# Chain123/RecGURU

Measured on AMD Instinct MI355X. Metric: user-sequences/sec (AE+GAN step), higher is better.
Workload: dtype bf16; 1 GPU; cross-domain RecGURU AE+GAN phase-2 iteration (5 critic + 1 generator update), two 100000-item domains; per_gpu_batch=4096, seq_len=200, d_model=128, n_head=4, n_blocks=3, d_ff=512, n_negs=30, user_lengths=U{5..220}, parallelism=dp1

## Files before the change

### include/recguru_hip.h

```cpp
#ifndef RECGURU_HIP_H
#define RECGURU_HIP_H
#include <stddef.h>
#include <stdint.h>
#ifdef __cplusplus
extern "C" {
#endif

#define RG_F32 0
#define RG_BF16 1
#define RG_X3 2

#define RG_ERR_INVALID (-1)
#define RG_ERR_UNSUPPORTED (-2)
#define RG_ERR_HIP (-3)

const char* rg_last_error(void);
int rg_version(void);

int rg_det_enabled(void);
int rg_det_set_arenas(void* fbase0, void* sbase0, unsigned long long bytes0, int bits0,
                      void* fbase1, void* sbase1, unsigned long long bytes1, int bits1);
int rg_det_fault(int clear);

#define RG_PRO_NONE 0
// ... 189 lines not shown
#define RG_CAST_SPLIT 4
int rg_cast(const float* src, void* dst, int R, int C, int transpose, int dtype, void* stream);
typedef struct {
  const float* src; void* dst;
  int R, C, ld, row_off, col_off, transpose;
} rg_cast_seg;
int rg_cast_multi(const rg_cast_seg* segs , const int* tiles , int ntiles,
                  int dtype, void* stream);

#define RG_LOSS_SAMPLED_CE 0
#define RG_LOSS_BPR 1
#define RG_LOSS_BPR_SAS 2
typedef struct {
  const void* h;
  const void* table;
  const int64_t* pos;
  const int64_t* neg;
  const float* mask;
  float* aux_tok;
  float* sums;
  const float* gout;
  void* dh; float* dE;
  long long ntok; int d; int k; int mode; long long skip_row;
} rg_item_loss_args;
int rg_item_loss_fwd(const rg_item_loss_args* args , int dtype, void* stream);
int rg_item_loss_bwd(const rg_item_loss_args* args , int dtype, void* stream);
size_t rg_item_loss_bwd_binned_workspace(long long ntok, int k, int d, long long table_rows);
int rg_item_loss_bwd_binned(const rg_item_loss_args* args , long long table_rows, void* workspace,
                            size_t workspace_bytes, int dtype, void* stream);
int rg_item_loss_train_supported(int k, int d);
int rg_item_loss_train(const rg_item_loss_args* args , float* coef, int dtype, void* stream);
int rg_item_loss_scatter_binned(const rg_item_loss_args* args , const float* coef, long long table_rows,
                                void* workspace, size_t workspace_bytes, int dtype, void* stream);
typedef struct {
  const void* h;
  const void* w;
  const int64_t* labels;
  const float* mask;
  const int* live16;
  float* lse;
  void* dh;
  float* partials;
  float* sums;
  const float* gout;
  float* dw;
  long long n; long long C; int d;
} rg_full_ce_args;
int rg_full_ce_supported(int d, int dtype);
int rg_full_ce_fwd(const rg_full_ce_args* args , int train, int dtype, void* stream);
int rg_full_ce_dw(const rg_full_ce_args* args , int dtype, void* stream);
typedef struct {
  const void* h;
  const void* table;
  const int64_t* labels;
  const int64_t* cand;
  const float* mask;
  const int* live16;
  const float* cand_bias;
  const float* pos_bias;
  void* wc;
  float* lse;
  void* dh;
  float* coef_pos;
  float* partials;
  float* sums;
  const float* gout;
// ... 174 lines not shown
```

### recguru_amd/csrc/loss.hip

```cpp
#include <stdlib.h>
#include "rg_common.hip.h"
#include "rg_det.hip.h"
#include "../../include/recguru_hip.h"

#define LW 4

#define RG_SAS_EPS 1e-24f
__device__ __forceinline__ float sigmoidf_(float x) { return 1.f / (1.f + __expf(-x)); }
__device__ __forceinline__ void bpr_value(int mode, float p, float nbar, float& loss, float& aux) {
  if (mode == RG_LOSS_BPR_SAS) {
    aux = nbar;
    loss = -(__logf(sigmoidf_(p) + RG_SAS_EPS) + __logf(1.f - sigmoidf_(nbar) + RG_SAS_EPS));
  } else {
    aux = p - nbar;
    loss = -__logf(sigmoidf_(aux));
  }
}
__device__ __forceinline__ float bpr_coef(int mode, int idx, float aux, float p, int k) {
  if (mode == RG_LOSS_BPR_SAS) {
    if (idx == 0) { const float sp = sigmoidf_(p); return -sp * (1.f - sp) / (sp + RG_SAS_EPS); }
    const float sn = sigmoidf_(aux);
    return sn * (1.f - sn) / (1.f - sn + RG_SAS_EPS) / (float)k;
  }
  const float sg = 1.f / (1.f + __expf(aux));
// ... 469 lines not shown
template <typename T>
static int launch(const rg_item_loss_args& a, bool bwd, hipStream_t s) {
  long long g = (a.ntok + LW - 1) / LW;
  if (g > 256 * 32) g = 256 * 32;
  dim3 grid((int)g), block(64 * LW);
#define RG_R(LPR)                                                                             \
  do {                                                                                        \
    if (bwd) hipLaunchKernelGGL((item_loss_bwd_rows_kernel<T, LPR, false>), grid, block, 0, s, a, (float*)nullptr);   \
    else hipLaunchKernelGGL((item_loss_fwd_rows_kernel<T, LPR>), grid, block, 0, s, a);       \
    RG_CHECK_LAUNCH();                                                                        \
    return 0;                                                                                 \
  } while (0)
  if (a.d == 64) RG_R(8);
  if (a.d == 128) RG_R(16);
  if (a.d == 256) RG_R(32);
#undef RG_R
#define RG_L(NPL)                                                                   \
  if (bwd) hipLaunchKernelGGL((item_loss_bwd_kernel<T, NPL>), grid, block, 0, s, a); \
  else hipLaunchKernelGGL((item_loss_fwd_kernel<T, NPL>), grid, block, 0, s, a)
  if (a.d <= 64) { RG_L(1); }
  else if (a.d <= 128) { RG_L(2); }
  else if (a.d <= 256) { RG_L(4); }
  else return rg_set_error_msg(RG_ERR_UNSUPPORTED, "item_loss: d > 256");
#undef RG_L
  RG_CHECK_LAUNCH();
  return 0;
}

#define RG_RPB 64
#define RG_RPB_LOG 6
#define RG_CHUNK 2048
#define RG_CHUNK_EMB 512
#define RG_MAXBINS 8192
#define RG_PPW 8192
#define RG_PPW_WIDE 65536

struct BinWs {
  float* c; int* hist; int* start; int* cursor; int* chunk_start;
  int* chunk_bin;
  int chunk;
  uint2* ent;
  int nbins;
  int ppw;
  int bin_log;
  const float* cscale;
  const float* lse;
  const float* count;
};

#define RG_PB 4
__device__ __forceinline__ void pair_items4(const rg_item_loss_args& a, long long p, long long p1, int n, long long (&it)[RG_PB]) {
  float mk[RG_PB];
#pragma unroll
  for (int u = 0; u < RG_PB; ++u) {
    const long long pc = min(p + 256 * u, p1 - 1);
    const long long t = (long long)((unsigned int)pc / (unsigned int)n);
    const int idx = (int)(pc - t * n);
    mk[u] = a.mask[t];
    const int64_t* __restrict__ src = idx == 0 ? a.pos + t : a.neg + t * a.k + (idx - 1);
    it[u] = *src;
  }
#pragma unroll
  for (int u = 0; u < RG_PB; ++u)
    if (p + 256 * u >= p1 || mk[u] == 0.f || it[u] == a.skip_row) it[u] = -1;
}

__global__ __launch_bounds__(256) void bin_count_kernel(rg_item_loss_args a, BinWs w) {
  extern __shared__ int lh[];
  const int n = a.k + 1;
  const long long npairs = a.ntok * n;
  for (int i = threadIdx.x; i < w.nbins; i += 256) lh[i] = 0;
  __syncthreads();
  const long long p0 = (long long)blockIdx.x * w.ppw, p1 = min(p0 + w.ppw, npairs);
  for (long long p = p0 + threadIdx.x; p < p1; p += 256 * RG_PB) {
    long long it[RG_PB];
    pair_items4(a, p, p1, n, it);
#pragma unroll
    for (int u = 0; u < RG_PB; ++u)
      if (it[u] >= 0) atomicAdd(&lh[it[u] >> w.bin_log], 1);
  }
  __syncthreads();
  for (int i = threadIdx.x; i < w.nbins; i += 256)
    if (lh[i]) atomicAdd(&w.hist[i], lh[i]);
}

__global__ __launch_bounds__(1024) void bin_scan_kernel(BinWs w) {
  __shared__ int wt[16], wtc[16];
  const int tid = threadIdx.x, lane = tid & 63, wv = tid >> 6;
  const int per = (w.nbins + 1023) / 1024;
  const int b0 = tid * per, b1 = min(b0 + per, w.nbins);
  int s = 0, sc = 0;
  for (int b = b0; b < b1; ++b) { s += w.hist[b]; sc += (w.hist[b] + w.chunk - 1) / w.chunk; }
  int is = s, isc = sc;
#pragma unroll
  for (int o = 1; o < 64; o <<= 1) {
    const int u = __shfl_up(is, o), uc = __shfl_up(isc, o);
    if (lane >= o) { is += u; isc += uc; }
  }
  if (lane == 63) { wt[wv] = is; wtc[wv] = isc; }
  __syncthreads();
  int base = 0, basec = 0;
  for (int i = 0; i < wv; ++i) { base += wt[i]; basec += wtc[i]; }
  if (tid == 1023) { w.start[w.nbins] = base + is; w.chunk_start[w.nbins] = basec + isc; }
  s = base + is - s; sc = basec + isc - sc;
  for (int b = b0; b < b1; ++b) {
    w.start[b] = s; w.cursor[b] = s; w.chunk_start[b] = sc;
    const int nc = (w.hist[b] + w.chunk - 1) / w.chunk;
    for (int j = 0; j < nc; ++j) w.chunk_bin[sc + j] = b;
    s += w.hist[b]; sc += nc;
  }
}

__global__ __launch_bounds__(256) void bin_fill_kernel(rg_item_loss_args a, BinWs w) {
  extern __shared__ int lh[];
  int* base = lh + w.nbins;
  const int n = a.k + 1;
  const long long npairs = a.ntok * n;
  const float gsc = w.cscale ? w.cscale[0] : 1.f;
  for (int i = threadIdx.x; i < w.nbins; i += 256) lh[i] = 0;
  __syncthreads();
  const long long p0 = (long long)blockIdx.x * w.ppw, p1 = min(p0 + w.ppw, npairs);
  for (long long p = p0 + threadIdx.x; p < p1; p += 256 * RG_PB) {
    long long it[RG_PB];
    pair_items4(a, p, p1, n, it);
#pragma unroll
    for (int u = 0; u < RG_PB; ++u)
      if (it[u] >= 0) atomicAdd(&lh[it[u] >> w.bin_log], 1);
  }
  __syncthreads();
  for (int i = threadIdx.x; i < w.nbins; i += 256) {
    const int cnt = lh[i];
    base[i] = cnt ? atomicAdd(&w.cursor[i], cnt) : 0;
    lh[i] = 0;
  }
  __syncthreads();
  for (long long p = p0 + threadIdx.x; p < p1; p += 256 * RG_PB) {
    long long it[RG_PB];
    float cv[RG_PB];
    pair_items4(a, p, p1, n, it);
#pragma unroll
    for (int u = 0; u < RG_PB; ++u) cv[u] = w.c[min(p + 256 * u, p1 - 1)];
    if (w.lse) {
      const float ic = 1.f / w.count[0];
#pragma unroll
      for (int u = 0; u < RG_PB; ++u) {
        const long long pc = min(p + 256 * u, p1 - 1);
        const long long t = (long long)((unsigned int)pc / (unsigned int)n);
        cv[u] = (__expf(cv[u] - w.lse[t]) - (pc - t * n == 0 ? 1.f : 0.f)) * a.mask[t] * ic;
      }
    }
#pragma unroll
    for (int u = 0; u < RG_PB; ++u) cv[u] *= gsc;
#pragma unroll
    for (int u = 0; u < RG_PB; ++u) {
      if (it[u] < 0) continue;
      const long long pu = p + 256 * u;
      const int b = (int)(it[u] >> w.bin_log);
      const int e = base[b] + atomicAdd(&lh[b], 1);
      w.ent[e] = make_uint2((((unsigned int)pu / (unsigned int)n) << w.bin_log) | (unsigned int)(it[u] & ((1 << w.bin_log) - 1)), __float_as_uint(cv[u]));
    }
  }
}

template <typename T, int LPR, bool DROP>
__global__ __launch_bounds__(256) void bin_accumulate_kernel(rg_item_loss_args a, BinWs w, long long table_rows, DropCfg drop) {
  constexpr int CH = DROP ? RG_CHUNK_EMB : RG_CHUNK;
  constexpr int G = 64 / LPR, D = LPR * 8, U = 4, EPT = CH / 256;
  extern __shared__ float sm[];
  float* acc = sm;
  int* st = reinterpret_cast<int*>(sm + RG_RPB * D);
  float* sc = reinterpret_cast<float*>(st + CH);
  __shared__ int cnt[RG_RPB], rstart[RG_RPB + 1];
// ... 252 lines not shown
        for (int u = 0; u < U; ++u)
#pragma unroll
          for (int j = 0; j < 8; ++j) s8[j] += c[u] * h[u][j];
      }
#pragma unroll
      for (int o = LPR; o < 64; o <<= 1)
#pragma unroll
        for (int j = 0; j < 8; ++j) s8[j] += __shfl_xor(s8[j], o);
      if (gi == 0) store8(myrow + 8 * li, s8);
      __builtin_amdgcn_fence(__ATOMIC_RELEASE, "wavefront");
      __builtin_amdgcn_wave_barrier();
      const long long row = (long long)bin * RB + r;
      if (row < table_rows) {
        float* __restrict__ dst = a.dE + row * D;
#pragma unroll
        for (int i = 0; i < D / 64; ++i) {
          const float v = myrow[lane + 64 * i];
          if (v != 0.f) { if (alone) dst[lane + 64 * i] += v; else atomicAdd(dst + lane + 64 * i, v); }
        }
      }
      __builtin_amdgcn_wave_barrier();
    }
    __syncthreads();
  }
}

static size_t align256(size_t x) { return (x + 255) & ~(size_t)255; }

static int bin_log_of(long long table_rows) {
  if ((table_rows + RG_RPB - 1) / RG_RPB <= RG_MAXBINS) return RG_RPB_LOG;
  if ((table_rows + RG_WIDE_RPB - 1) / RG_WIDE_RPB <= RG_MAXBINS) return RG_WIDE_LOG;
  return 0;
}
extern "C" size_t rg_item_loss_bwd_binned_workspace(long long ntok, int k, int d, long long table_rows) {
  if (RG_DET) return 0;
  const int bl = bin_log_of(table_rows);
  if (!bl) return 0;
  const long long nbins = (table_rows + (1LL << bl) - 1) >> bl;
  const long long npairs = ntok * (k + 1);
  if (!(d == 64 || d == 128 || d == 256) || npairs >= (1LL << 31) || ntok <= 0 || ntok >= (1LL << (32 - bl))) return 0;
  return align256(npairs * 4) + align256(npairs * 8) + align256((nbins + 1) * 4) * 4 + align256((nbins + npairs / RG_CHUNK_EMB + 1) * 4);
}

template <typename T>
static int launch_binned(const rg_item_loss_args& a, const float* coef, void* ws, size_t ws_bytes, long long table_rows, hipStream_t s,
                         const DropCfg* drop = nullptr) {
  const int n = a.k + 1;
  const long long npairs = a.ntok * n;
  const size_t need = rg_item_loss_bwd_binned_workspace(a.ntok, a.k, a.d, table_rows);
  if (!need) return rg_set_error_msg(RG_ERR_UNSUPPORTED, "item_loss_bwd_binned: needs d in {64,128,256}, <= 8192 bins of 64 (or 256) rows, < 2^31 pairs, < 2^26 (2^24) positions");
  if (!ws || ws_bytes < need) return rg_set_error_msg(RG_ERR_INVALID, "item_loss_bwd_binned: workspace too small");
  BinWs w;
  w.bin_log = bin_log_of(table_rows);
  const bool wide = w.bin_log == RG_WIDE_LOG;
  if (wide && drop) return rg_set_error_msg(RG_ERR_UNSUPPORTED, "embed_scatter_bwd_binned: tables of more than 524288 rows take the atomic form");
  w.nbins = (int)((table_rows + (1LL << w.bin_log) - 1) >> w.bin_log);
  char* p = reinterpret_cast<char*>(ws);
  w.c = coef ? const_cast<float*>(coef) : reinterpret_cast<float*>(p); p += align256(npairs * 4);
  w.cscale = coef ? a.gout : nullptr;
  w.lse = coef ? a.aux_tok : nullptr;
  w.count = a.sums ? a.sums + 1 : nullptr;
  if (w.lse && !w.count) return rg_set_error_msg(RG_ERR_INVALID, "item_loss_scatter_binned: aux_tok (lse of raw logits) needs sums");
  w.chunk = drop ? RG_CHUNK_EMB : (wide ? RG_CHUNK_WIDE : RG_CHUNK);
  w.ent = reinterpret_cast<uint2*>(p); p += align256(npairs * 8);
  const size_t ib = align256((size_t)(w.nbins + 1) * 4);
  w.hist = reinterpret_cast<int*>(p); p += ib;
  w.start = reinterpret_cast<int*>(p); p += ib;
  w.cursor = reinterpret_cast<int*>(p); p += ib;
  w.chunk_start = reinterpret_cast<int*>(p); p += ib;
  w.chunk_bin = reinterpret_cast<int*>(p);
  hipError_t e = hipMemsetAsync(w.hist, 0, ib, s);
  if (e != hipSuccess) return rg_set_error(e, "item_loss_bwd_binned(memset)");
  long long g = (a.ntok + LW - 1) / LW;
  if (g > 256 * 32) g = 256 * 32;
  if (coef) {}
  else if (a.d == 64) hipLaunchKernelGGL((item_loss_bwd_rows_kernel<T, 8, true>), dim3((int)g), dim3(64 * LW), 0, s, a, w.c);
  else if (a.d == 128) hipLaunchKernelGGL((item_loss_bwd_rows_kernel<T, 16, true>), dim3((int)g), dim3(64 * LW), 0, s, a, w.c);
  else hipLaunchKernelGGL((item_loss_bwd_rows_kernel<T, 32, true>), dim3((int)g), dim3(64 * LW), 0, s, a, w.c);
  w.ppw = w.nbins > 4096 ? RG_PPW_WIDE : RG_PPW;
  const int gp = (int)((npairs + w.ppw - 1) / w.ppw);
  hipLaunchKernelGGL(bin_count_kernel, dim3(gp), dim3(256), (size_t)w.nbins * 4, s, a, w);
  hipLaunchKernelGGL(bin_scan_kernel, dim3(1), dim3(1024), 0, s, w);
  hipFuncSetAttribute(reinterpret_cast<const void*>(bin_fill_kernel), hipFuncAttributeMaxDynamicSharedMemorySize, w.nbins * 8);
  hipLaunchKernelGGL(bin_fill_kernel, dim3(gp), dim3(256), (size_t)w.nbins * 8, s, a, w);
  if (wide) {
    const size_t smw = (size_t)RG_CHUNK_WIDE * 8 + (size_t)4 * a.d * 4;
#define RG_ACCW(LPR)                                                                                                 \
  do {                                                                                                               \
    hipFuncSetAttribute(reinterpret_cast<const void*>(bin_accumulate_wide_kernel<T, LPR>), hipFuncAttributeMaxDynamicSharedMemorySize, (int)smw); \
    hipLaunchKernelGGL((bin_accumulate_wide_kernel<T, LPR>), dim3(256 * 2), dim3(256), smw, s, a, w, table_rows);      \
  } while (0)
    if (a.d == 64) RG_ACCW(8);
    else if (a.d == 128) RG_ACCW(16);
    else RG_ACCW(32);
#undef RG_ACCW
    RG_CHECK_LAUNCH();
    return 0;
  }
  const size_t smem = (size_t)RG_RPB * a.d * 4 + (size_t)(drop ? RG_CHUNK_EMB : RG_CHUNK) * 8;
  const int ga = 256 * (int)(smem <= 40 * 1024 ? 4 : (smem <= 52 * 1024 ? 3 : (smem <= 80 * 1024 ? 2 : 1)));
#define RG_ACC1(LPR, DR)                                                                                            \
  do {                                                                                                              \
    hipFuncSetAttribute(reinterpret_cast<const void*>(bin_accumulate_kernel<T, LPR, DR>), hipFuncAttributeMaxDynamicSharedMemorySize, (int)smem); \
    hipLaunchKernelGGL((bin_accumulate_kernel<T, LPR, DR>), dim3(ga), dim3(256), smem, s, a, w, table_rows, dc);      \
  } while (0)
#define RG_ACC(LPR) do { if (drop) RG_ACC1(LPR, true); else RG_ACC1(LPR, false); } while (0)
  const DropCfg dc = drop ? *drop : make_drop(0.f, 0);
  if (a.d == 64) RG_ACC(8);
  else if (a.d == 128) RG_ACC(16);
  else RG_ACC(32);
#undef RG_ACC1
#undef RG_ACC
  RG_CHECK_LAUNCH();
  return 0;
}

extern "C" int rg_item_loss_bwd_binned(const rg_item_loss_args* a, long long table_rows, void* workspace, size_t workspace_bytes,
// ... 29 lines not shown
    else if (a.d == 128) hipLaunchKernelGGL((item_loss_train_online2_kernel<T, 16>), grid, block, 0, s, a, coef);
    else hipLaunchKernelGGL((item_loss_train_online2_kernel<T, 32>), grid, block, 0, s, a, coef);
    RG_CHECK_LAUNCH();
    return 0;
  }
#define RG_TR(LPR)                                                                                           \
  do {                                                                                                       \
    if (nit == 1) hipLaunchKernelGGL((item_loss_train_rows_kernel<T, LPR, 1>), grid, block, 0, s, a, coef);  \
    else if (nit == 2) hipLaunchKernelGGL((item_loss_train_rows_kernel<T, LPR, 2>), grid, block, 0, s, a, coef); \
    else hipLaunchKernelGGL((item_loss_train_rows_kernel<T, LPR, 4>), grid, block, 0, s, a, coef);           \
  } while (0)
  if (a.d == 64) RG_TR(8);
  else if (a.d == 128) RG_TR(16);
  else RG_TR(32);
#undef RG_TR
  RG_CHECK_LAUNCH();
  return 0;
}

extern "C" int rg_item_loss_train(const rg_item_loss_args* a, float* coef, int dtype, void* stream) {
  if (!a || a->ntok <= 0) return 0;
  if (dtype == RG_BF16) return launch_train<__bf16>(*a, coef, (hipStream_t)stream);
  if (dtype == RG_F32) return launch_train<float>(*a, coef, (hipStream_t)stream);
  return rg_set_error_msg(RG_ERR_INVALID, "item_loss_train: bad dtype");
}

extern "C" int rg_item_loss_scatter_binned(const rg_item_loss_args* a, const float* coef, long long table_rows, void* workspace,
                                           size_t workspace_bytes, int dtype, void* stream) {
  if (!a || a->ntok <= 0) return 0;
  if (!coef || !a->gout) return rg_set_error_msg(RG_ERR_INVALID, "item_loss_scatter_binned: coef and gout are required");
  if (dtype == RG_BF16) return launch_binned<__bf16>(*a, coef, workspace, workspace_bytes, table_rows, (hipStream_t)stream);
  if (dtype == RG_F32) return launch_binned<float>(*a, coef, workspace, workspace_bytes, table_rows, (hipStream_t)stream);
  return rg_set_error_msg(RG_ERR_INVALID, "item_loss_scatter_binned: bad dtype");
}

extern "C" size_t rg_embed_scatter_binned_workspace(long long ntok, int d, long long table_rows) {
  if (bin_log_of(table_rows) != RG_RPB_LOG) return 0;
  return rg_item_loss_bwd_binned_workspace(ntok, 0, d, table_rows);
}
extern "C" int rg_embed_scatter_bwd_binned(const void* dx, const int64_t* ids, const float* mask, float* dE, long long ntok, int d,
                                           long long table_rows, long long skip_row, float drop_p, unsigned long long seed,
                                           void* workspace, size_t workspace_bytes, int dtype, void* stream) {
  if (ntok <= 0) return 0;
  if (!dx || !ids || !mask || !dE) return rg_set_error_msg(RG_ERR_INVALID, "embed_scatter_bwd_binned: dx, ids, mask and dE are required");
  rg_item_loss_args a = {};
  a.h = dx; a.pos = ids; a.mask = mask; a.dE = dE; a.ntok = ntok; a.d = d; a.k = 0; a.skip_row = skip_row;
  const DropCfg drop = make_drop(drop_p, seed);
  if (dtype == RG_BF16) return launch_binned<__bf16>(a, mask, workspace, workspace_bytes, table_rows, (hipStream_t)stream, &drop);
  if (dtype == RG_F32) return launch_binned<float>(a, mask, workspace, workspace_bytes, table_rows, (hipStream_t)stream, &drop);
  return rg_set_error_msg(RG_ERR_INVALID, "embed_scatter_bwd_binned: bad dtype");
}

template <typename T, int LPR>
__global__ __launch_bounds__(64 * LW) void rank_scores_kernel(rg_rank_args a) {
  constexpr int G = 64 / LPR;
  const int lane = threadIdx.x & 63, wave = threadIdx.x >> 6;
  const int gi = lane / LPR, li = lane % LPR;
  const T* __restrict__ H = reinterpret_cast<const T*>(a.h);
  const T* __restrict__ E = reinterpret_cast<const T*>(a.table);
  const int d = a.d, n = a.C + 1;
  for (int b = blockIdx.x * LW + wave; b < a.B; b += gridDim.x * LW) {
    float h[8];
    load8(h, H + (size_t)b * d + 8 * li);
    const long long tgt = a.target[b];
    float s0;
    {
// ... 77 lines not shown
```

### recguru_amd/hip.py

```python
import ctypes
import os

import torch

_HERE = os.path.dirname(os.path.abspath(__file__))
DETERMINISTIC = os.environ.get("RG_DETERMINISTIC", "0") not in ("", "0")
LIB_PATH = os.environ.get("RG_HIP_LIB") or os.path.join(_HERE, "librecguru_hip_det.so" if DETERMINISTIC else "librecguru_hip.so")
_lib = None

F32, BF16, X3 = 0, 1, 2
SPLIT_OPERANDS = False
PRO_NONE, PRO_GELU = 0, 1
EPI_NONE, EPI_RELU, EPI_MUL_POSMASK, EPI_GELU_GRAD, EPI_ADD, EPI_RESID_LN, EPI_DROP_GELU = 0, 1, 2, 3, 4, 5, 6

c_p, c_i, c_f, c_l = ctypes.c_void_p, ctypes.c_int, ctypes.c_float, ctypes.c_int64
c_u64 = ctypes.c_uint64


class GemmNtArgs(ctypes.Structure):
    _fields_ = [("A", c_p), ("lda", c_i), ("W", c_p), ("ldw", c_i), ("bias", c_p), ("C", c_p), ("ldc", c_i),
                ("c_is_f32", c_i), ("M", c_i), ("N", c_i), ("K", c_i), ("prologue", c_i), ("epilogue", c_i),
                ("aux", c_p), ("ldaux", c_i), ("gamma", c_p), ("beta", c_p), ("rowmask", c_p),
                ("rstd_out", c_p), ("ln_eps", c_f), ("debug_ablate", c_i), ("epi_scale", c_f),
                ("epi_nonzero_scale", c_f), ("drop_p", c_f), ("drop_seed", c_u64), ("live16", c_p),
# ... 35 lines not shown
class FfnBwdArgs(ctypes.Structure):
    _fields_ = [("dl2", c_p), ("dz", c_p), ("h1", c_p), ("W2t", c_p), ("W1t", c_p), ("dh1", c_p), ("dy", c_p),
                ("M", c_i), ("d", c_i), ("dff", c_i), ("w_packed", c_i), ("nz_scale", c_f), ("live16", c_p),
                ("ln_dout", c_p), ("ln_out", c_p), ("ln_rstd", c_p), ("ln_gamma", c_p), ("ln_beta", c_p), ("ln_rowmask", c_p),
                ("dl2_out", c_p), ("ln_dgamma", c_p), ("ln_dbeta", c_p), ("ln_partials", c_p),
                ("ln_drop_p", c_f), ("ln_drop_seed", c_u64)]


class AttnOutBwdArgs(ctypes.Structure):
    _fields_ = [("dy", c_p), ("y", c_p), ("rstd", c_p), ("gamma", c_p), ("beta", c_p), ("rowmask", c_p), ("Wot", c_p),
                ("dz", c_p), ("dctx", c_p), ("dgamma", c_p), ("dbeta", c_p), ("ln_partials", c_p),
                ("M", c_i), ("d", c_i), ("P", c_i), ("w_packed", c_i), ("live16", c_p)]


class AttnOutBwdCrossArgs(ctypes.Structure):
    _fields_ = [("dy2", c_p), ("y2", c_p), ("rstd_c", c_p), ("cgamma", c_p), ("cbeta", c_p),
                ("y1", c_p), ("rstd1", c_p), ("gamma1", c_p), ("beta1", c_p), ("rowmask", c_p), ("Wot", c_p),
                ("dy1", c_p), ("dz", c_p), ("dctx", c_p),
                ("dcgamma", c_p), ("dcbeta", c_p), ("dz_colsum", c_p), ("dgamma1", c_p), ("dbeta1", c_p), ("partials", c_p),
                ("M", c_i), ("d", c_i), ("P", c_i), ("w_packed", c_i), ("live16", c_p)]


SYMBOLS = ["rg_last_error", "rg_version", "rg_gemm_nt", "rg_gemm_tn", "rg_attn_fwd", "rg_attn_bwd",
           "rg_embed_pe_fwd", "rg_embed_pe_fwd_rows", "rg_embed_scatter_bwd", "rg_ln_bwd", "rg_bcast_add_ln", "rg_seq_sum", "rg_colsum",
           "rg_outer_posmask", "rg_interpolate", "rg_gp_penalty", "rg_sum", "rg_adam", "rg_cast",
           "rg_item_loss_fwd", "rg_item_loss_bwd", "rg_post_attn_fwd",
           "rg_attn_lastq_fwd", "rg_attn_lastq_bwd",
           "rg_cross_drop_scale", "rg_seq_wsum", "rg_gemm_nt_plan", "rg_gemm_tn_plan", "rg_gemm_tn_workspace", "rg_gemm_tn_layer", "rg_gemm_tn_layer_supported", "rg_gemm_tn_layer_workspace", "rg_ln_bwd_workspace", "rg_cast_multi",
           "rg_item_loss_bwd_binned_workspace", "rg_item_loss_bwd_binned", "rg_adam_multi", "rg_rank_scores",
           "rg_assemble_batch", "rg_sample_negatives", "rg_sample_negatives_alias", "rg_dropout", "rg_cross_rows", "rg_live_tiles",
           "rg_adam_multi_dev", "rg_disc_rows", "rg_disc_supported", "rg_attn_fwd_x_supported", "rg_pad_mask", "rg_last_rows",
           "rg_ffn_bwd_data", "rg_ffn_bwd_data_supported", "rg_ffn_bwd_ln_workspace", "rg_first_live",
           "rg_attn_out_bwd", "rg_attn_out_bwd_workspace", "rg_attn_out_bwd_cross", "rg_attn_out_bwd_cross_workspace",
           "rg_item_loss_train_supported", "rg_item_loss_train", "rg_item_loss_scatter_binned", "rg_scale_dev",
           "rg_attn_lastq_x_supported", "rg_attn_lastq_x_fwd", "rg_attn_lastq_x_bwd", "rg_attn_lastq_xf_fwd", "rg_attn_lastq_xf_bwd",
           "rg_embed_scatter_binned_workspace", "rg_embed_scatter_bwd_binned", "rg_embed_pe_fwd_split", "rg_mse",
           "rg_dropout_gelu", "rg_add_drop_ln", "rg_cross_add_ln", "rg_embed_pe_fwd2",
           "rg_det_enabled", "rg_det_set_arenas", "rg_det_fault",
           "rg_full_ce_supported", "rg_full_ce_fwd", "rg_full_ce_dw",
           "rg_shared_ce_supported", "rg_shared_ce_bwd_workspace", "rg_shared_ce_fwd", "rg_shared_ce_bwd",
           "rg_topk_workspace", "rg_topk_scores", "rg_topk_list_workspace", "rg_topk_list",
           "rg_grad_sqnorm_multi", "rg_adam_multi_dev2",
           "rg_pos_grad_workspace", "rg_pos_grad"]
LOSS_SAMPLED_CE, LOSS_BPR, LOSS_BPR_SAS = 0, 1, 2
c_ll = ctypes.c_longlong


class LnBwdArgs(ctypes.Structure):
    _fields_ = [("dy", c_p), ("y", c_p), ("rstd", c_p), ("gamma", c_p), ("beta", c_p), ("rowmask", c_p),
                ("dz", c_p), ("dgamma", c_p), ("dbeta", c_p), ("M", c_ll), ("N", c_i), ("ld", c_i),
                ("dz_drop", c_p), ("drop_p", c_f), ("drop_seed", c_u64), ("live16", c_p), ("dz_colsum", c_p), ("partials", c_p)]


class ItemLossArgs(ctypes.Structure):
    _fields_ = [("h", c_p), ("table", c_p), ("pos", c_p), ("neg", c_p), ("mask", c_p), ("aux_tok", c_p),
                ("sums", c_p), ("gout", c_p), ("dh", c_p), ("dE", c_p), ("ntok", c_ll), ("d", c_i), ("k", c_i),
                ("mode", c_i), ("skip_row", c_ll)]


def _check_screened(path):
    if os.environ.get("RG_ALLOW_UNSCREENED") or os.environ.get("RG_HIP_LIB"):
        return
    info_path = os.path.join(_HERE, "build", "BUILD_INFO_det.json" if os.path.basename(path) == "librecguru_hip_det.so" else "BUILD_INFO.json")
    try:
        import json
        with open(info_path) as f:
            info = json.load(f)
# ... 855 lines not shown

def item_loss_train_supported(k, d):
    return int(lib().rg_item_loss_train_supported(int(k), int(d)))


@_det_accum(sums="S")
def item_loss_train(h, table, pos, neg, mask, k, mode, sums, lse=None):
    ntok, d = h.shape
    assert h.is_contiguous() and table.is_contiguous() and table.dtype == h.dtype
    assert pos.dtype == torch.int64 and neg.dtype == torch.int64 and pos.numel() == ntok and neg.numel() == ntok * k
    coef = torch.empty(ntok * (k + 1), device=h.device, dtype=torch.float32)
    dh = torch.empty_like(h)
    a = ItemLossArgs(_p(h), _p(table), _p(pos), _p(neg), _p(mask), _p(lse), _p(sums), None, _p(dh), None, ntok, d, k,
                     mode, -1)
    _check(lib().rg_item_loss_train(ctypes.byref(a), _vp(coef), dt_of(h), _stream()), "rg_item_loss_train")
    return coef, dh


def item_loss_scatter_binned(h, table_rows, pos, neg, mask, k, coef, gout, dE, skip_row=-1, lse=None, sums=None):
    ntok, d = h.shape
    need = item_loss_bwd_binned_supported(ntok, k, d, table_rows)
    if not need:
        raise RuntimeError("item_loss_scatter_binned: unsupported shape (d=%d, rows=%d, k=%d)" % (d, table_rows, k))
    ws = _BIN_WS.get(h.device)
    if ws is None or ws.numel() < need:
        ws = torch.empty(need, device=h.device, dtype=torch.uint8)
        _BIN_WS[h.device] = ws
    a = ItemLossArgs(_p(h), None, _p(pos), _p(neg), _p(mask), _p(lse), _p(sums), _p(gout), None, _p(dE), ntok, d, k, 0,
                     skip_row)
    _check(lib().rg_item_loss_scatter_binned(ctypes.byref(a), _vp(coef), c_ll(table_rows), _vp(ws), ctypes.c_size_t(need),
                                             dt_of(h), _stream()), "rg_item_loss_scatter_binned")


class FullCeArgs(ctypes.Structure):
    _fields_ = [("h", c_p), ("w", c_p), ("labels", c_p), ("mask", c_p), ("live16", c_p), ("lse", c_p), ("dh", c_p),
                ("partials", c_p), ("sums", c_p), ("gout", c_p), ("dw", c_p), ("n", c_ll), ("C", c_ll), ("d", c_i)]


def _full_ce_code(h):
    return BF16 if h.dtype == torch.bfloat16 else X3


def full_ce_supported(d, h):
    return bool(lib().rg_full_ce_supported(int(d), _full_ce_code(h)))


def full_ce_fwd(h, w, labels, mask, live, sums, train=True):
    n, d = h.shape
    assert h.is_contiguous() and w.is_contiguous() and w.dtype == h.dtype and w.shape[1] == d
    assert labels.dtype == torch.int64 and labels.numel() == n and mask.dtype == torch.float32 and mask.numel() == n
    lse = torch.empty(n, device=h.device, dtype=torch.float32)
    dh = torch.empty_like(h) if train else None
    partials = torch.empty((n + 15) // 16, device=h.device, dtype=torch.float32)
    a = FullCeArgs(_p(h), _p(w), _p(labels), _p(mask), _p(live), _p(lse), _p(dh), _p(partials), _p(sums), None, None,
                   n, w.shape[0], d)
    _check(lib().rg_full_ce_fwd(ctypes.byref(a), int(bool(train)), _full_ce_code(h), _stream()), "rg_full_ce_fwd")
    return lse, dh


def full_ce_dw(h, w, labels, mask, live, lse, sums, gout, dw):
    n, d = h.shape
    assert dw.dtype == torch.float32 and dw.is_contiguous() and tuple(dw.shape) == tuple(w.shape)
    a = FullCeArgs(_p(h), _p(w), _p(labels), _p(mask), _p(live), _p(lse), None, None, _p(sums), _p(gout), _p(dw),
                   n, w.shape[0], d)
    _check(lib().rg_full_ce_dw(ctypes.byref(a), _full_ce_code(h), _stream()), "rg_full_ce_dw")
    return dw
# ... 514 lines not shown
    return ("attn_fwd_kernel<bf16,x-input>", 4.0 * B * H * L * L * 32 + 2.0 * B * L * d * P3,
            B * L * (d + P3 // 3) * _esize(x) + P3 * d * _esize(x))


def _work_ffn_bwd(dl2, dz, h1, *a, **k):
    src = k["ln"][0] if k.get("ln") is not None else dl2
    M, d = src.shape
    dff = h1.shape[1]
    return ("ffn_bwd_data_kernel<%s>" % _tn(src), 4.0 * M * d * dff,
            M * ((4 if k.get("ln") is not None else 3) * d + 2 * dff) * _esize(src))


def _work_lastq_x_fwd(x, q_last, *a, **k):
    B, L, d = x.shape
    return "attn_lastq_x_fwd_kernel", B * (4 * 2.0 * L * d * 2 + 4 * 2.0 * 32 * d * 2), B * L * d * _esize(x) + 2 * B * d * _esize(x)


def _work_lastq_x_bwd(x, q_last, *a, **k):
    B, L, d = x.shape
    return "attn_lastq_x_bwd_kernel", B * (4 * 2.0 * L * d * 5 + 4 * 2.0 * 32 * d * 3), 2 * B * L * d * _esize(x) + 11 * B * d * _esize(x)


def _work_item_loss_train(h, table, pos, neg, mask, k, mode, *a, **kw):
    n, d = h.shape
    nl = float(mask.sum())
    return ("item_loss_train_rows_kernel", 4.0 * nl * (k + 1) * d,
            nl * (k + 2) * d * _esize(table) + n * d * _esize(table) + nl * (k + 1) * 12 + n * 4)


def _work_item_loss_scatter(h, table_rows, pos, neg, mask, k, coef, gout, dE, *a, **kw):
    n, d = h.shape
    nl = float(mask.sum())
    pairs = nl * (k + 1)
    return "item_loss_scatter_binned_kernel", 2.0 * pairs * d, pairs * (d * _esize(h) + 2 * 12 + 2 * 8)


def _work_gemm_tn_layer(probs):
    fl, by, refs = [], [], []
    for i, pr in enumerate(probs):
        if pr is None:
            continue
        Y, X, dW, colsum, live = pr
        T, N1, N2 = Y.shape[0], Y.shape[1], X.shape[1]
        fl.append(2.0 * T * N1 * N2)
        by.append(T * (N1 + N2) * _esize(Y) + N1 * N2 * 4)
        refs.append(live)
    x3 = any(pr is not None and pr[0].dtype == torch.float32 for pr in probs)
    return "gemm_tn_layer_x3_kernel" if x3 else "gemm_tn_layer_kernel", fl, by, refs


def _work_attn_out_bwd(dy, y, rstd, *a, **k):
    M, d = dy.shape
    return "attn_out_bwd_kernel", 2.0 * M * d * d, 4 * M * d * _esize(dy) + M * 4


def _work_attn_out_bwd_cross(dy2, y2, rstd_c, *a, **k):
    M, d = dy2.shape
    return "attn_out_bwd_cross_kernel", 2.0 * M * d * d, 6 * M * d * _esize(dy2) + 3 * M * 4


def _work_ln_bwd(dy, y, rstd, *a, **k):
    M, N = dy.shape
    return "ln_bwd_kernel", 0.0, 3 * M * N * _esize(dy) + M * 4


def _work_full_ce_fwd(h, w, labels, mask, live, sums, train=True):
    n, d = h.shape
# ... 100 lines not shown
```

Baseline: 880,500 user-sequences/sec.

## Replace atomic bin cursors with per-workgroup count matrix and column scan

For the 64-row bin case, the counting sort now writes each workgroup's per-bin histogram into a matrix. A column-wise exclusive scan over that matrix gives each workgroup fixed offsets, so the fill pass no longer takes global atomics on shared cursors and does not have to recount. Sort kernels use 1024 threads and the pairs-per-workgroup is sized so the matrix stays within a 32 MB cap. A standalone rg_bin_sort entry is also exposed, at the cost of extra workspace and an extra scan launch.

```diff
diff --git a/include/recguru_hip.h b/include/recguru_hip.h
--- a/include/recguru_hip.h
+++ b/include/recguru_hip.h
@@ -245,6 +245,9 @@
 int rg_item_loss_train(const rg_item_loss_args* args , float* coef, int dtype, void* stream);
 int rg_item_loss_scatter_binned(const rg_item_loss_args* args , const float* coef, long long table_rows,
                                 void* workspace, size_t workspace_bytes, int dtype, void* stream);
+int rg_bin_sort(const rg_item_loss_args* args , const float* coef, long long table_rows, int ppw, void* workspace,
+                size_t workspace_bytes, size_t* need, long long* ent_off, long long* start_off, int* nbins, int* bin_log,
+                void* stream);
 typedef struct {
   const void* h;
   const void* w;
diff --git a/recguru_amd/csrc/loss.hip b/recguru_amd/csrc/loss.hip
--- a/recguru_amd/csrc/loss.hip
+++ b/recguru_amd/csrc/loss.hip
@@ -525,11 +525,15 @@
 #define RG_CHUNK 2048
 #define RG_CHUNK_EMB 512
 #define RG_MAXBINS 8192
+#define RG_SORT_T 1024
 #define RG_PPW 8192
+#define RG_MAT_BYTES (32u << 20)
 #define RG_PPW_WIDE 65536
 
 struct BinWs {
-  float* c; int* hist; int* start; int* cursor; int* chunk_start;
+  float* c; int* hist; int* start; int* chunk_start;
+  int* mat;
+  int* cursor;
   int* chunk_bin;
   int chunk;
   uint2* ent;
@@ -542,11 +546,12 @@
 };
 
 #define RG_PB 4
-__device__ __forceinline__ void pair_items4(const rg_item_loss_args& a, long long p, long long p1, int n, long long (&it)[RG_PB]) {
-  float mk[RG_PB];
-#pragma unroll
-  for (int u = 0; u < RG_PB; ++u) {
-    const long long pc = min(p + 256 * u, p1 - 1);
+template <int NT, int PB>
+__device__ __forceinline__ void pair_items(const rg_item_loss_args& a, long long p, long long p1, int n, long long (&it)[PB]) {
+  float mk[PB];
+#pragma unroll
+  for (int u = 0; u < PB; ++u) {
+    const long long pc = min(p + NT * u, p1 - 1);
     const long long t = (long long)((unsigned int)pc / (unsigned int)n);
     const int idx = (int)(pc - t * n);
     mk[u] = a.mask[t];
@@ -554,11 +559,61 @@
     it[u] = *src;
   }
 #pragma unroll
-  for (int u = 0; u < RG_PB; ++u)
-    if (p + 256 * u >= p1 || mk[u] == 0.f || it[u] == a.skip_row) it[u] = -1;
-}
-
-__global__ __launch_bounds__(256) void bin_count_kernel(rg_item_loss_args a, BinWs w) {
+  for (int u = 0; u < PB; ++u)
+    if (p + NT * u >= p1 || mk[u] == 0.f || it[u] == a.skip_row) it[u] = -1;
+}
+
+__global__ __launch_bounds__(RG_SORT_T) void bin_count_kernel(rg_item_loss_args a, BinWs w) {
+  extern __shared__ int lh[];
+  const int n = a.k + 1;
+  const long long npairs = a.ntok * n;
+  for (int i = threadIdx.x; i < w.nbins; i += RG_SORT_T) lh[i] = 0;
+  __syncthreads();
+  const long long p0 = (long long)blockIdx.x * w.ppw, p1 = min(p0 + w.ppw, npairs);
+  for (long long p = p0 + threadIdx.x; p < p1; p += RG_SORT_T * RG_PB) {
+    long long it[RG_PB];
+    pair_items<RG_SORT_T, RG_PB>(a, p, p1, n, it);
+#pragma unroll
+    for (int u = 0; u < RG_PB; ++u)
+      if (it[u] >= 0) atomicAdd(&lh[it[u] >> RG_RPB_LOG], 1);
+  }
+  __syncthreads();
+  int* __restrict__ row = w.mat + (size_t)blockIdx.x * w.nbins;
+  for (int i = threadIdx.x; i < w.nbins; i += RG_SORT_T) row[i] = lh[i];
+}
+
+#define RG_CS_BINS 8
+#define RG_CS_SEG 128
+__global__ __launch_bounds__(RG_CS_BINS * RG_CS_SEG) void bin_colscan_kernel(BinWs w, int nwg) {
+  __shared__ int tot[RG_CS_SEG][RG_CS_BINS];
+  const int bl = threadIdx.x % RG_CS_BINS, sg = threadIdx.x / RG_CS_BINS;
+  const int b = blockIdx.x * RG_CS_BINS + bl;
+  const bool live = b < w.nbins;
+  const int per = (nwg + RG_CS_SEG - 1) / RG_CS_SEG;
+  const int r0 = min(sg * per, nwg), r1 = min(r0 + per, nwg);
+  int* __restrict__ col = w.mat + b;
+  int s = 0;
+  if (live)
+    for (int r = r0; r < r1; ++r) s += col[(size_t)r * w.nbins];
+  tot[sg][bl] = s;
+  __syncthreads();
+  int run = 0;
+  for (int i = 0; i < sg; ++i) run += tot[i][bl];
+  if (live) {
+    int r = r0;
+    for (; r + 8 <= r1; r += 8) {
+      int v[8];
+#pragma unroll
+      for (int u = 0; u < 8; ++u) v[u] = col[(size_t)(r + u) * w.nbins];
+#pragma unroll
+      for (int u = 0; u < 8; ++u) { col[(size_t)(r + u) * w.nbins] = run; run += v[u]; }
+    }
+    for (; r < r1; ++r) { const int v = col[(size_t)r * w.nbins]; col[(size_t)r * w.nbins] = run; run += v; }
+    if (sg == RG_CS_SEG - 1) w.hist[b] = run;
+  }
+}
+
+__global__ __launch_bounds__(256) void bin_count_wide_kernel(rg_item_loss_args a, BinWs w) {
   extern __shared__ int lh[];
   const int n = a.k + 1;
   const long long npairs = a.ntok * n;
@@ -567,7 +622,7 @@
   const long long p0 = (long long)blockIdx.x * w.ppw, p1 = min(p0 + w.ppw, npairs);
   for (long long p = p0 + threadIdx.x; p < p1; p += 256 * RG_PB) {
     long long it[RG_PB];
-    pair_items4(a, p, p1, n, it);
+    pair_items<256, RG_PB>(a, p, p1, n, it);
 #pragma unroll
     for (int u = 0; u < RG_PB; ++u)
       if (it[u] >= 0) atomicAdd(&lh[it[u] >> w.bin_log], 1);
@@ -597,14 +652,51 @@
   if (tid == 1023) { w.start[w.nbins] = base + is; w.chunk_start[w.nbins] = basec + isc; }
   s = base + is - s; sc = basec + isc - sc;
   for (int b = b0; b < b1; ++b) {
-    w.start[b] = s; w.cursor[b] = s; w.chunk_start[b] = sc;
+    w.start[b] = s; w.chunk_start[b] = sc;
+    if (w.cursor) w.cursor[b] = s;
     const int nc = (w.hist[b] + w.chunk - 1) / w.chunk;
     for (int j = 0; j < nc; ++j) w.chunk_bin[sc + j] = b;
     s += w.hist[b]; sc += nc;
   }
 }
 
-__global__ __launch_bounds__(256) void bin_fill_kernel(rg_item_loss_args a, BinWs w) {
+__global__ __launch_bounds__(RG_SORT_T) void bin_fill_kernel(rg_item_loss_args a, BinWs w) {
+  extern __shared__ int lh[];
+  const int n = a.k + 1;
+  const long long npairs = a.ntok * n;
+  const float gsc = w.cscale ? w.cscale[0] : 1.f;
+  const int* __restrict__ row = w.mat + (size_t)blockIdx.x * w.nbins;
+  for (int i = threadIdx.x; i < w.nbins; i += RG_SORT_T) lh[i] = w.start[i] + row[i];
+  __syncthreads();
+  const long long p0 = (long long)blockIdx.x * w.ppw, p1 = min(p0 + w.ppw, npairs);
+  for (long long p = p0 + threadIdx.x; p < p1; p += RG_SORT_T * RG_PB) {
+    long long it[RG_PB];
+    float cv[RG_PB];
+    pair_items<RG_SORT_T, RG_PB>(a, p, p1, n, it);
+#pragma unroll
+    for (int u = 0; u < RG_PB; ++u) cv[u] = w.c[min(p + RG_SORT_T * u, p1 - 1)];
+    if (w.lse) {
+      const float ic = 1.f / w.count[0];
+#pragma unroll
+      for (int u = 0; u < RG_PB; ++u) {
+        const long long pc = min(p + RG_SORT_T * u, p1 - 1);
+        const long long t = (long long)((unsigned int)pc / (unsigned int)n);
+        cv[u] = (__expf(cv[u] - w.lse[t]) - (pc - t * n == 0 ? 1.f : 0.f)) * a.mask[t] * ic;
+      }
+    }
+#pragma unroll
+    for (int u = 0; u < RG_PB; ++u) cv[u] *= gsc;
+#pragma unroll
+    for (int u = 0; u < RG_PB; ++u) {
+      if (it[u] < 0) continue;
+      const long long pu = p + RG_SORT_T * u;
+      const int e = atomicAdd(&lh[it[u] >> RG_RPB_LOG], 1);
+      w.ent[e] = make_uint2((((unsigned int)pu / (unsigned int)n) << RG_RPB_LOG) | (unsigned int)(it[u] & (RG_RPB - 1)), __float_as_uint(cv[u]));
+    }
+  }
+}
+
+__global__ __launch_bounds__(256) void bin_fill_wide_kernel(rg_item_loss_args a, BinWs w) {
   extern __shared__ int lh[];
   int* base = lh + w.nbins;
   const int n = a.k + 1;
@@ -615,7 +707,7 @@
   const long long p0 = (long long)blockIdx.x * w.ppw, p1 = min(p0 + w.ppw, npairs);
   for (long long p = p0 + threadIdx.x; p < p1; p += 256 * RG_PB) {
     long long it[RG_PB];
-    pair_items4(a, p, p1, n, it);
+    pair_items<256, RG_PB>(a, p, p1, n, it);
 #pragma unroll
     for (int u = 0; u < RG_PB; ++u)
       if (it[u] >= 0) atomicAdd(&lh[it[u] >> w.bin_log], 1);
@@ -630,7 +722,7 @@
   for (long long p = p0 + threadIdx.x; p < p1; p += 256 * RG_PB) {
     long long it[RG_PB];
     float cv[RG_PB];
-    pair_items4(a, p, p1, n, it);
+    pair_items<256, RG_PB>(a, p, p1, n, it);
 #pragma unroll
     for (int u = 0; u < RG_PB; ++u) cv[u] = w.c[min(p + 256 * u, p1 - 1)];
     if (w.lse) {
@@ -949,14 +1041,60 @@
   if ((table_rows + RG_WIDE_RPB - 1) / RG_WIDE_RPB <= RG_MAXBINS) return RG_WIDE_LOG;
   return 0;
 }
+static int binned_ppw(long long npairs, int nbins) {
+  int ppw = RG_PPW;
+  while ((npairs + ppw - 1) / ppw * nbins * 4 > (long long)RG_MAT_BYTES) ppw *= 2;
+  return ppw;
+}
+
+static size_t bin_carve(BinWs& w, void* ws, long long npairs) {
+  size_t off = 0;
+  auto take = [&](size_t bytes) { char* q = ws ? reinterpret_cast<char*>(ws) + off : nullptr; off += align256(bytes); return q; };
+  const size_t ib = (size_t)(w.nbins + 1) * 4;
+  w.c = reinterpret_cast<float*>(take(npairs * 4));
+  w.ent = reinterpret_cast<uint2*>(take(npairs * 8));
+  w.hist = reinterpret_cast<int*>(take(ib));
+  w.start = reinterpret_cast<int*>(take(ib));
+  w.chunk_start = reinterpret_cast<int*>(take(ib));
+  w.chunk_bin = reinterpret_cast<int*>(take((size_t)(w.nbins + npairs / RG_CHUNK_EMB + 1) * 4));
+  w.cursor = w.mat = nullptr;
+  if (w.bin_log == RG_RPB_LOG) w.mat = reinterpret_cast<int*>(take((size_t)((npairs + w.ppw - 1) / w.ppw) * w.nbins * 4));
+  else w.cursor = reinterpret_cast<int*>(take(ib));
+  return off;
+}
+
+static bool bin_shape(BinWs& w, long long ntok, int k, long long table_rows, int ppw) {
+  w.bin_log = bin_log_of(table_rows);
+  const long long npairs = ntok * (k + 1);
+  if (!w.bin_log || npairs >= (1LL << 31) || ntok <= 0 || ntok >= (1LL << (32 - w.bin_log))) return false;
+  w.nbins = (int)((table_rows + (1LL << w.bin_log) - 1) >> w.bin_log);
+  w.ppw = ppw ? ppw : (w.bin_log == RG_RPB_LOG ? binned_ppw(npairs, w.nbins) : (w.nbins > 4096 ? RG_PPW_WIDE : RG_PPW));
+  return true;
+}
+
 extern "C" size_t rg_item_loss_bwd_binned_workspace(long long ntok, int k, int d, long long table_rows) {
   if (RG_DET) return 0;
-  const int bl = bin_log_of(table_rows);
-  if (!bl) return 0;
-  const long long nbins = (table_rows + (1LL << bl) - 1) >> bl;
-  const long long npairs = ntok * (k + 1);
-  if (!(d == 64 || d == 128 || d == 256) || npairs >= (1LL << 31) || ntok <= 0 || ntok >= (1LL << (32 - bl))) return 0;
-  return align256(npairs * 4) + align256(npairs * 8) + align256((nbins + 1) * 4) * 4 + align256((nbins + npairs / RG_CHUNK_EMB + 1) * 4);
+  BinWs w;
+  if (!(d == 64 || d == 128 || d == 256) || !bin_shape(w, ntok, k, table_rows, 0)) return 0;
+  return bin_carve(w, nullptr, ntok * (k + 1));
+}
+
+static int launch_sort(const rg_item_loss_args& a, const BinWs& w, long long npairs, hipStream_t s) {
+  const int gp = (int)((npairs + w.ppw - 1) / w.ppw);
+  if (w.bin_log == RG_RPB_LOG) {
+    hipLaunchKernelGGL(bin_count_kernel, dim3(gp), dim3(RG_SORT_T), (size_t)w.nbins * 4, s, a, w);
+    hipLaunchKernelGGL(bin_colscan_kernel, dim3((w.nbins + RG_CS_BINS - 1) / RG_CS_BINS), dim3(RG_CS_BINS * RG_CS_SEG), 0, s, w, gp);
+    hipLaunchKernelGGL(bin_scan_kernel, dim3(1), dim3(1024), 0, s, w);
+    hipLaunchKernelGGL(bin_fill_kernel, dim3(gp), dim3(RG_SORT_T), (size_t)w.nbins * 4, s, a, w);
+    return 0;
+  }
+  hipError_t e = hipMemsetAsync(w.hist, 0, align256((size_t)(w.nbins + 1) * 4), s);
+  if (e != hipSuccess) return rg_set_error(e, "item_loss_bwd_binned(memset)");
+  hipLaunchKernelGGL(bin_count_wide_kernel, dim3(gp), dim3(256), (size_t)w.nbins * 4, s, a, w);
+  hipLaunchKernelGGL(bin_scan_kernel, dim3(1), dim3(1024), 0, s, w);
+  hipFuncSetAttribute(reinterpret_cast<const void*>(bin_fill_wide_kernel), hipFuncAttributeMaxDynamicSharedMemorySize, w.nbins * 8);
+  hipLaunchKernelGGL(bin_fill_wide_kernel, dim3(gp), dim3(256), (size_t)w.nbins * 8, s, a, w);
+  return 0;
 }
 
 template <typename T>
@@ -968,38 +1106,23 @@
   if (!need) return rg_set_error_msg(RG_ERR_UNSUPPORTED, "item_loss_bwd_binned: needs d in {64,128,256}, <= 8192 bins of 64 (or 256) rows, < 2^31 pairs, < 2^26 (2^24) positions");
   if (!ws || ws_bytes < need) return rg_set_error_msg(RG_ERR_INVALID, "item_loss_bwd_binned: workspace too small");
   BinWs w;
-  w.bin_log = bin_log_of(table_rows);
+  bin_shape(w, a.ntok, a.k, table_rows, 0);
   const bool wide = w.bin_log == RG_WIDE_LOG;
   if (wide && drop) return rg_set_error_msg(RG_ERR_UNSUPPORTED, "embed_scatter_bwd_binned: tables of more than 524288 rows take the atomic form");
-  w.nbins = (int)((table_rows + (1LL << w.bin_log) - 1) >> w.bin_log);
-  char* p = reinterpret_cast<char*>(ws);
-  w.c = coef ? const_cast<float*>(coef) : reinterpret_cast<float*>(p); p += align256(npairs * 4);
+  bin_carve(w, ws, npairs);
+  if (coef) w.c = const_cast<float*>(coef);
   w.cscale = coef ? a.gout : nullptr;
   w.lse = coef ? a.aux_tok : nullptr;
   w.count = a.sums ? a.sums + 1 : nullptr;
   if (w.lse && !w.count) return rg_set_error_msg(RG_ERR_INVALID, "item_loss_scatter_binned: aux_tok (lse of raw logits) needs sums");
   w.chunk = drop ? RG_CHUNK_EMB : (wide ? RG_CHUNK_WIDE : RG_CHUNK);
-  w.ent = reinterpret_cast<uint2*>(p); p += align256(npairs * 8);
-  const size_t ib = align256((size_t)(w.nbins + 1) * 4);
-  w.hist = reinterpret_cast<int*>(p); p += ib;
-  w.start = reinterpret_cast<int*>(p); p += ib;
-  w.cursor = reinterpret_cast<int*>(p); p += ib;
-  w.chunk_start = reinterpret_cast<int*>(p); p += ib;
-  w.chunk_bin = reinterpret_cast<int*>(p);
-  hipError_t e = hipMemsetAsync(w.hist, 0, ib, s);
-  if (e != hipSuccess) return rg_set_error(e, "item_loss_bwd_binned(memset)");
   long long g = (a.ntok + LW - 1) / LW;
   if (g > 256 * 32) g = 256 * 32;
   if (coef) {}
   else if (a.d == 64) hipLaunchKernelGGL((item_loss_bwd_rows_kernel<T, 8, true>), dim3((int)g), dim3(64 * LW), 0, s, a, w.c);
   else if (a.d == 128) hipLaunchKernelGGL((item_loss_bwd_rows_kernel<T, 16, true>), dim3((int)g), dim3(64 * LW), 0, s, a, w.c);
   else hipLaunchKernelGGL((item_loss_bwd_rows_kernel<T, 32, true>), dim3((int)g), dim3(64 * LW), 0, s, a, w.c);
-  w.ppw = w.nbins > 4096 ? RG_PPW_WIDE : RG_PPW;
-  const int gp = (int)((npairs + w.ppw - 1) / w.ppw);
-  hipLaunchKernelGGL(bin_count_kernel, dim3(gp), dim3(256), (size_t)w.nbins * 4, s, a, w);
-  hipLaunchKernelGGL(bin_scan_kernel, dim3(1), dim3(1024), 0, s, w);
-  hipFuncSetAttribute(reinterpret_cast<const void*>(bin_fill_kernel), hipFuncAttributeMaxDynamicSharedMemorySize, w.nbins * 8);
-  hipLaunchKernelGGL(bin_fill_kernel, dim3(gp), dim3(256), (size_t)w.nbins * 8, s, a, w);
+  if (int rc = launch_sort(a, w, npairs, s)) return rc;
   if (wide) {
     const size_t smw = (size_t)RG_CHUNK_WIDE * 8 + (size_t)4 * a.d * 4;
 #define RG_ACCW(LPR)                                                                                                 \
@@ -1095,6 +1218,33 @@
   if (dtype == RG_BF16) return launch_binned<__bf16>(*a, coef, workspace, workspace_bytes, table_rows, (hipStream_t)stream);
   if (dtype == RG_F32) return launch_binned<float>(*a, coef, workspace, workspace_bytes, table_rows, (hipStream_t)stream);
   return rg_set_error_msg(RG_ERR_INVALID, "item_loss_scatter_binned: bad dtype");
+}
+
+extern "C" int rg_bin_sort(const rg_item_loss_args* a, const float* coef, long long table_rows, int ppw, void* workspace,
+                           size_t workspace_bytes, size_t* need, long long* ent_off, long long* start_off, int* nbins, int* bin_log,
+                           void* stream) {
+  if (RG_DET) return rg_set_error_msg(RG_ERR_UNSUPPORTED, "bin_sort: the deterministic build does not offer the binned path");
+  if (!a || !coef || !need || !ent_off || !start_off || !nbins || !bin_log || ppw < 0)
+    return rg_set_error_msg(RG_ERR_INVALID, "bin_sort: args, coef and the outputs are required; ppw >= 0");
+  BinWs w;
+  if (!bin_shape(w, a->ntok, a->k, table_rows, ppw)) return rg_set_error_msg(RG_ERR_UNSUPPORTED, "bin_sort: unsupported shape");
+  const long long npairs = a->ntok * (a->k + 1);
+  *need = bin_carve(w, nullptr, npairs);
+  *nbins = w.nbins; *bin_log = w.bin_log;
+  if (!workspace) return 0;
+  if (workspace_bytes < *need) return rg_set_error_msg(RG_ERR_INVALID, "bin_sort: workspace too small");
+  bin_carve(w, workspace, npairs);
+  *ent_off = reinterpret_cast<char*>(w.ent) - reinterpret_cast<char*>(workspace);
+  *start_off = reinterpret_cast<char*>(w.start) - reinterpret_cast<char*>(workspace);
+  w.c = const_cast<float*>(coef);
+  w.cscale = a->gout;
+  w.lse = a->aux_tok;
+  w.count = a->sums ? a->sums + 1 : nullptr;
+  if (w.lse && !w.count) return rg_set_error_msg(RG_ERR_INVALID, "bin_sort: aux_tok (lse of raw logits) needs sums");
+  w.chunk = w.bin_log == RG_RPB_LOG ? RG_CHUNK : RG_CHUNK_WIDE;
+  if (int rc = launch_sort(*a, w, npairs, (hipStream_t)stream)) return rc;
+  RG_CHECK_LAUNCH();
+  return 0;
 }
 
 extern "C" size_t rg_embed_scatter_binned_workspace(long long ntok, int d, long long table_rows) {
diff --git a/recguru_amd/hip.py b/recguru_amd/hip.py
--- a/recguru_amd/hip.py
+++ b/recguru_amd/hip.py
@@ -91,7 +91,7 @@
            "rg_adam_multi_dev", "rg_disc_rows", "rg_disc_supported", "rg_attn_fwd_x_supported", "rg_pad_mask", "rg_last_rows",
            "rg_ffn_bwd_data", "rg_ffn_bwd_data_supported", "rg_ffn_bwd_ln_workspace", "rg_first_live",
            "rg_attn_out_bwd", "rg_attn_out_bwd_workspace", "rg_attn_out_bwd_cross", "rg_attn_out_bwd_cross_workspace",
-           "rg_item_loss_train_supported", "rg_item_loss_train", "rg_item_loss_scatter_binned", "rg_scale_dev",
+           "rg_item_loss_train_supported", "rg_item_loss_train", "rg_item_loss_scatter_binned", "rg_bin_sort", "rg_scale_dev",
            "rg_attn_lastq_x_supported", "rg_attn_lastq_x_fwd", "rg_attn_lastq_x_bwd", "rg_attn_lastq_xf_fwd", "rg_attn_lastq_xf_bwd",
            "rg_embed_scatter_binned_workspace", "rg_embed_scatter_bwd_binned", "rg_embed_pe_fwd_split", "rg_mse",
            "rg_dropout_gelu", "rg_add_drop_ln", "rg_cross_add_ln", "rg_embed_pe_fwd2",
@@ -1013,6 +1013,22 @@
                                              dt_of(h), _stream()), "rg_item_loss_scatter_binned")
 
 
+def bin_sort(pos, neg, mask, k, coef, skip_row, table_rows, ppw=0, lse=None, sums=None, gout=None):
+    ntok = mask.numel()
+    a = ItemLossArgs(None, None, _p(pos), _p(neg), _p(mask), _p(lse), _p(sums), _p(gout), None, None, ntok, 0, k, 0, skip_row)
+    need, eo, so = ctypes.c_size_t(0), c_ll(0), c_ll(0)
+    nb, bl = ctypes.c_int(0), ctypes.c_int(0)
+    outs = (ctypes.byref(need), ctypes.byref(eo), ctypes.byref(so), ctypes.byref(nb), ctypes.byref(bl))
+    _check(lib().rg_bin_sort(ctypes.byref(a), _vp(coef), c_ll(table_rows), int(ppw), None, ctypes.c_size_t(0), *outs, _stream()),
+           "rg_bin_sort")
+    ws = torch.empty(need.value, device=mask.device, dtype=torch.uint8)
+    _check(lib().rg_bin_sort(ctypes.byref(a), _vp(coef), c_ll(table_rows), int(ppw), _vp(ws), ctypes.c_size_t(need.value), *outs,
+                             _stream()), "rg_bin_sort")
+    start = ws[so.value:so.value + 4 * (nb.value + 1)].view(torch.int32)
+    ent = ws[eo.value:eo.value + 8 * ntok * (k + 1)].view(torch.int32).view(-1, 2)
+    return start, ent, bl.value
+
+
 class FullCeArgs(ctypes.Structure):
     _fields_ = [("h", c_p), ("w", c_p), ("labels", c_p), ("mask", c_p), ("live16", c_p), ("lse", c_p), ("dh", c_p),
                 ("partials", c_p), ("sums", c_p), ("gout", c_p), ("dw", c_p), ("n", c_ll), ("C", c_ll), ("d", c_i)]
@@ -1593,7 +1609,7 @@
     n, d = h.shape
     nl = float(mask.sum())
     pairs = nl * (k + 1)
-    return "item_loss_scatter_binned_kernel", 2.0 * pairs * d, pairs * (d * _esize(h) + 2 * 12 + 2 * 8)
+    return "item_loss_scatter_binned_kernel", 2.0 * pairs * d, pairs * (d * _esize(h) + 2 * 8 + 4 + 2 * 8)
 
 
 def _work_gemm_tn_layer(probs):
```

New measurement: 885,400 user-sequences/sec, median of 6. No clear change (+0.6%).
